# dronefreak/CABiNet

Measured on AMD Instinct MI355X. Metric: 1024x1024 images/sec fwd+bwd (CABiNet-MobileNetV3-Large), higher is better.
Workload: dtype f32; 1 GPU; BASELINE configs[2]: CABiNet-MobileNetV3-Large, 8x3x1024x1024 synthetic 8-class per GPU, fwd + 2x OhemCE + bwd + grad all-reduce + SGD step, HIP CAB/FFM kernels, fp32, random-init (model seed 0, gamma=0.5); per_gpu_batch=8, global_batch=8, n_classes=8, parallelism=dp1, miopen_find_mode=FAST

## Files before the change

cabinet_amd/csrc/conv3x3_s2.hip:

```cpp
#include "common.hpp"
#include "slab_sum.hpp"

namespace cabinet {

struct C3Shape {
    int B, H, W, Ho, Wo;
};

static C3Shape c3_shape(int B, int H, int W) { return C3Shape{B, H, W, (H - 1) / 2 + 1, (W - 1) / 2 + 1}; }

constexpr int CW_C = 64;
constexpr int CW_TW = 32;
constexpr int CW_IW = 2 * CW_TW + 1;
constexpr int CW_XP = 3 * CW_IW;
constexpr int CW_DLD = CW_TW + 1;
constexpr int CW_SLAB = CW_C * CW_C * 9;
constexpr int CW_TARGET_WG = 512;
constexpr int CW_MIN_ROWS = 4;

struct C3Plan {
    int tiles_x, strips, rows_per;
};

static C3Plan cw_plan(const C3Shape& s) {
    C3Plan p;
    p.tiles_x = ceil_div(s.Wo, CW_TW);
    const long per = (long)s.B * p.tiles_x;
    long strips = CW_TARGET_WG / per;
    const int cap = ceil_div(s.Ho, CW_MIN_ROWS);
    if (strips > cap) strips = cap;
    if (strips < 1) strips = 1;
    p.rows_per = ceil_div(s.Ho, (int)strips);
    p.strips = ceil_div(s.Ho, p.rows_per);
    return p;
}

__global__ __launch_bounds__(256, 2) void conv3x3s2_wgrad64_kernel(const float* __restrict__ dy, const float* __restrict__ x,
                                                                 C3Shape s, int tiles_x, int strips, int rows_per,
                                                                 float* __restrict__ slabs) {
    extern __shared__ __attribute__((aligned(16))) float smem[];
    float* xs = smem;
    float* dys = xs + CW_C * CW_XP;
    const int tid = threadIdx.x, wave = tid >> 6, lane = tid & 63, li = lane & 31, h = lane >> 5;
    int bi = blockIdx.x;
    const int tx = bi % tiles_x;
    bi /= tiles_x;
    const int strip = bi % strips, b = bi / strips;
    const int oy_begin = strip * rows_per, oy_end = min(s.Ho, oy_begin + rows_per);
    const int ox0 = tx * CW_TW, ix0 = 2 * ox0 - 1;
    const int ch = wave & 1, cj = wave >> 1;

    f32x16 acc[9];
#pragma unroll
    for (int t = 0; t < 9; ++t)
#pragma unroll
        for (int r = 0; r < 16; ++r) acc[t][r] = 0.f;

    const float* xb = x + (size_t)b * CW_C * s.H * s.W;
    const float* dyb = dy + (size_t)b * CW_C * s.Ho * s.Wo;
    const float* arow = dys + (32 * ch + li) * CW_DLD + h;
    const float* brow = xs + (32 * cj + li) * CW_XP + 2 * h;
    for (int oy = oy_begin; oy < oy_end; ++oy) {
        const int iy0 = 2 * oy - 1;
        __syncthreads();
        for (int i = tid; i < CW_C * CW_XP; i += 256) {
            const int ci = i / CW_XP, r = i - ci * CW_XP, yy = r / CW_IW, xx = r - yy * CW_IW;
            const int iy = iy0 + yy, ix = ix0 + xx;
            xs[i] = (iy >= 0 && iy < s.H && ix >= 0 && ix < s.W) ? xb[((size_t)ci * s.H + iy) * s.W + ix] : 0.f;
        }
        for (int i = tid; i < CW_C * CW_TW; i += 256) {
            const int co = i >> 5, c = i & 31, ox = ox0 + c;
            dys[co * CW_DLD + c] = ox < s.Wo ? dyb[((size_t)co * s.Ho + oy) * s.Wo + ox] : 0.f;
        }
        __syncthreads();
#pragma unroll
        for (int c0 = 0; c0 < CW_TW; c0 += 2) {
            const float a = arow[c0];
#pragma unroll
            for (int ky = 0; ky < 3; ++ky)
#pragma unroll
                for (int kx = 0; kx < 3; ++kx)
                    acc[3 * ky + kx] = mfma32(a, brow[ky * CW_IW + 2 * c0 + kx], acc[3 * ky + kx]);
        }
    }
    float* slab = slabs + (size_t)blockIdx.x * CW_SLAB;
#pragma unroll
    for (int r = 0; r < 16; ++r) {
        const int co = 32 * ch + acc_row(r) + 4 * h, ci = 32 * cj + li;
        float* p = slab + (co * CW_C + ci) * 9;
#pragma unroll
        for (int t = 0; t < 9; ++t) p[t] = acc[t][r];
    }
}

constexpr int CF_CI = 3, CF_CO = 16, CF_KK = CF_CI * 9;
constexpr int CF_TH = 4, CF_TW = 32;
constexpr int CF_IH = 2 * CF_TH + 1, CF_IW = 2 * CF_TW + 1;
constexpr int CF_PATCH = CF_CI * CF_IH * CF_IW;
constexpr int CF_DLD = CF_TH * CF_TW + 1;
constexpr int CF_SLAB = CF_CO * CF_KK;

__global__ __launch_bounds__(256) void conv3x3s2_wgrad_3_16_kernel(const float* __restrict__ dy, const float* __restrict__ x,
                                                                  C3Shape s, int tiles_x, float* __restrict__ slabs) {
    __shared__ __attribute__((aligned(16))) float dys[32 * CF_DLD];
    __shared__ float xs[CF_PATCH];
    __shared__ float red[4][CF_CO][32];
    const int tid = threadIdx.x, wave = tid >> 6, lane = tid & 63, li = lane & 31, h = lane >> 5;
    const int strips_y = (s.Ho + CF_TH - 1) / CF_TH;
    const int b = blockIdx.x / strips_y, oy0 = (blockIdx.x - b * strips_y) * CF_TH;
    const int kk = li < CF_KK ? li : 0;
    const int ko = ((kk / 9) * CF_IH + (kk % 9) / 3) * CF_IW + kk % 3;
    f32x16 acc;
#pragma unroll
    for (int r = 0; r < 16; ++r) acc[r] = 0.f;
    for (int i = tid; i < 16 * CF_DLD; i += 256) dys[16 * CF_DLD + i] = 0.f;
    const float* xb = x + (size_t)b * CF_CI * s.H * s.W;
    const float* dyb = dy + (size_t)b * CF_CO * s.Ho * s.Wo;
    const int iy0 = 2 * oy0 - 1;
    for (int t = 0; t < tiles_x; ++t) {
        const int ox0 = t * CF_TW, ix0 = 2 * ox0 - 1;
        __syncthreads();
        for (int i = tid; i < CF_PATCH; i += 256) {
            const int ci = i / (CF_IH * CF_IW), r = i - ci * CF_IH * CF_IW, yy = r / CF_IW, xx = r - yy * CF_IW;
            const int iy = iy0 + yy, ix = ix0 + xx;
            xs[i] = (iy >= 0 && iy < s.H && ix >= 0 && ix < s.W) ? xb[((size_t)ci * s.H + iy) * s.W + ix] : 0.f;
        }
        for (int i = tid; i < CF_CO * CF_TH * CF_TW; i += 256) {
            const int co = i / (CF_TH * CF_TW), p = i - co * (CF_TH * CF_TW), r = p / CF_TW, c = p - r * CF_TW;
            const int oy = oy0 + r, ox = ox0 + c;
            dys[co * CF_DLD + p] = (oy < s.Ho && ox < s.Wo) ? dyb[((size_t)co * s.Ho + oy) * s.Wo + ox] : 0.f;
        }
        __syncthreads();
        const float* drow = dys + li * CF_DLD + 32 * wave + h;
        const float* prow = xs + ko + 2 * wave * CF_IW + 2 * h;
#pragma unroll
        for (int c0 = 0; c0 < 32; c0 += 2) acc = mfma32(drow[c0], prow[2 * c0], acc);
    }
#pragma unroll
    for (int r = 0; r < 16; ++r) {
        const int co = acc_row(r) + 4 * h;
        if (co < CF_CO) red[wave][co][li] = acc[r];
    }
    __syncthreads();
    float* slab = slabs + (size_t)blockIdx.x * CF_SLAB;
    for (int i = tid; i < CF_SLAB; i += 256) {
        const int co = i / CF_KK, k = i - co * CF_KK;
        slab[i] = ((red[0][co][k] + red[1][co][k]) + red[2][co][k]) + red[3][co][k];
    }
}

typedef float f32x4v __attribute__((ext_vector_type(4)));
__device__ __forceinline__ f32x4v mfma16(float a, float b, f32x4v c) { return __builtin_amdgcn_mfma_f32_16x16x4f32(a, b, c, 0, 0, 0); }

constexpr int CD_NT = 64;
constexpr int CD_RP = 72;
constexpr int CD_CP = 2 * CD_RP;

__host__ __device__ constexpr int cd_par(int k) { return k == 1 ? 0 : 1; }
__host__ __device__ constexpr int cd_shift(int k) { return k == 0 ? 1 : 0; }

__global__ __launch_bounds__(256, 2) void conv3x3s2_dgrad64_kernel(const float* __restrict__ dy, const float* __restrict__ w,
                                                                 C3Shape s, int tiles_n, int strips, int rows_per,
                                                                 float* __restrict__ dx) {
    __shared__ __attribute__((aligned(16))) float dys[CW_C * CD_CP];
    const int tid = threadIdx.x, wave = tid >> 6, lane = tid & 63, lc = lane & 15, lk = lane >> 4;
    int bi = blockIdx.x;
    const int tn = bi % tiles_n;
    bi /= tiles_n;
    const int strip = bi % strips, b = bi / strips;
    const int m_begin = strip * rows_per, m_end = min(s.Ho, m_begin + rows_per);
    const int n0 = tn * CD_NT;
    const int ci0 = 16 * wave;

    float wr[9][16];
#pragma unroll
    for (int t = 0; t < 9; ++t)
#pragma unroll
        for (int ks = 0; ks < 16; ++ks) wr[t][ks] = w[((4 * ks + lk) * CW_C + ci0 + lc) * 9 + t];

    const float* dyb = dy + (size_t)b * CW_C * s.Ho * s.Wo;
    float* dxb = dx + ((size_t)b * CW_C + ci0 + 4 * lk) * s.H * s.W;
    const float* brow = dys + lk * CD_CP + lc;
    const bool pair_ok = (s.W & 1) == 0;
    for (int m = m_begin; m < m_end; ++m) {
        __syncthreads();
        for (int i = tid; i < CW_C * 2 * (CD_NT + 1); i += 256) {
            const int co = i / (2 * (CD_NT + 1)), r = i - co * 2 * (CD_NT + 1), rr = r / (CD_NT + 1), c = r - rr * (CD_NT + 1);
            const int oy = m + rr, ox = n0 + c;
            dys[co * CD_CP + rr * CD_RP + c] = (oy < s.Ho && ox < s.Wo) ? dyb[((size_t)co * s.Ho + oy) * s.Wo + ox] : 0.f;
        }
        __syncthreads();
#pragma unroll 1
        for (int ng = 0; ng < CD_NT / 16 && n0 + 16 * ng < s.Wo; ++ng) {
            f32x4v acc[2][2];
#pragma unroll
            for (int i = 0; i < 2; ++i)
#pragma unroll
                for (int j = 0; j < 2; ++j) acc[i][j] = f32x4v{0.f, 0.f, 0.f, 0.f};
            const float* bp = brow + 16 * ng;
#pragma unroll
            for (int ky = 0; ky < 3; ++ky)
#pragma unroll
                for (int kx = 0; kx < 3; ++kx) {
                    f32x4v p0 = {0.f, 0.f, 0.f, 0.f}, p1 = {0.f, 0.f, 0.f, 0.f};
                    const float* bt = bp + cd_shift(ky) * CD_RP + cd_shift(kx);
#pragma unroll
                    for (int ks = 0; ks < 16; ks += 2) {
                        p0 = mfma16(wr[3 * ky + kx][ks], bt[4 * ks * CD_CP], p0);
                        p1 = mfma16(wr[3 * ky + kx][ks + 1], bt[4 * (ks + 1) * CD_CP], p1);
                    }
                    acc[cd_par(ky)][cd_par(kx)] += p0 + p1;
                }
            const int ix = 2 * (n0 + 16 * ng + lc);
#pragma unroll
            for (int rp = 0; rp < 2; ++rp) {
                const int iy = 2 * m + rp;
                if (iy < s.H && ix < s.W) {
#pragma unroll
                    for (int r = 0; r < 4; ++r) {
                        float* p = dxb + ((size_t)r * s.H + iy) * s.W + ix;
                        if (pair_ok) {
                            *reinterpret_cast<f32x2*>(p) = f32x2{acc[rp][0][r], acc[rp][1][r]};
                        } else {
                            p[0] = acc[rp][0][r];
                            if (ix + 1 < s.W) p[1] = acc[rp][1][r];
                        }
                    }
                }
            }
        }
    }
}

bool conv3x3s2_supported(int Ci, int Co) { return (Ci == CW_C && Co == CW_C) || (Ci == CF_CI && Co == CF_CO); }

static C3Plan cd_plan(const C3Shape& s) {
    C3Plan p;
    p.tiles_x = ceil_div(s.Wo, CD_NT);
    const long per = (long)s.B * p.tiles_x;
    long strips = CW_TARGET_WG / per;
    if (strips > s.Ho) strips = s.Ho;
    if (strips < 1) strips = 1;
    p.rows_per = ceil_div(s.Ho, (int)strips);
    p.strips = ceil_div(s.Ho, p.rows_per);
    return p;
}

long long conv3x3s2_dgrad_workgroups(int B, int H, int W) {
    const C3Shape s = c3_shape(B, H, W);
    const long long per = (long long)B * ceil_div(s.Wo, CD_NT);
    if (per > (1ll << 30)) return per;
    const C3Plan p = cd_plan(s);
    return per * p.strips;
}

hipError_t conv3x3s2_dgrad_run(const float* dy, const float* w, int B, int H, int W, float* dx, hipStream_t stream) {
    const C3Shape s = c3_shape(B, H, W);
    const C3Plan p = cd_plan(s);
    hipLaunchKernelGGL(conv3x3s2_dgrad64_kernel, dim3(B * p.tiles_x * p.strips), dim3(256), 0, stream, dy, w, s, p.tiles_x,
                       p.strips, p.rows_per, dx);
    return hipGetLastError();
}

long long conv3x3s2_wgrad_slabs(int B, int Ci, int H, int W) {
    const C3Shape s = c3_shape(B, H, W);
    if (Ci == CF_CI) return (long long)B * ceil_div(s.Ho, CF_TH);
    const long long tiles_x = ceil_div(s.Wo, CW_TW);
    if ((long long)B * tiles_x > (1ll << 30)) return (long long)B * tiles_x;
    const C3Plan p = cw_plan(s);
    return (long long)B * p.tiles_x * p.strips;
}

size_t conv3x3s2_wgrad_workspace(int B, int Ci, int H, int W) {
    return align_up((size_t)conv3x3s2_wgrad_slabs(B, Ci, H, W) * (Ci == CF_CI ? CF_SLAB : CW_SLAB) * sizeof(float), 256);
}

hipError_t conv3x3s2_wgrad_run(const float* dy, const float* x, int B, int Ci, int H, int W, float* dw, void* ws,
                               hipStream_t stream) {
    const C3Shape s = c3_shape(B, H, W);
    float* slabs = static_cast<float*>(ws);
    const int nslab = (int)conv3x3s2_wgrad_slabs(B, Ci, H, W);
    if (Ci == CF_CI) {
        hipLaunchKernelGGL(conv3x3s2_wgrad_3_16_kernel, dim3(nslab), dim3(256), 0, stream, dy, x, s, ceil_div(s.Wo, CF_TW),
                           slabs);
    } else {
        const C3Plan p = cw_plan(s);
        const size_t lds = (size_t)(CW_C * CW_XP + CW_C * CW_DLD) * sizeof(float);
        static lds_attr_mask mask{0};
        if (hipError_t e = ensure_dynamic_lds(reinterpret_cast<const void*>(conv3x3s2_wgrad64_kernel), lds, mask); e != hipSuccess)
            return e;
        hipLaunchKernelGGL(conv3x3s2_wgrad64_kernel, dim3(nslab), dim3(256), lds, stream, dy, x, s, p.tiles_x, p.strips,
                           p.rows_per, slabs);
    }
    hipError_t e = hipGetLastError();
    if (e != hipSuccess) return e;
    slab_sum_launch(slabs, nslab, Ci == CF_CI ? CF_SLAB : CW_SLAB, dw, stream);
    return hipGetLastError();
}

}
```

cabinet_amd/csrc/stem_conv.hip:

```cpp
#include "act.hpp"
#include "common.hpp"
#include "slab_sum.hpp"

namespace cabinet {

constexpr int ST_K = 7, ST_S = 2, ST_PAD = 3, ST_CI = 3, ST_CO = 64;
constexpr int ST_KK = ST_CI * ST_K * ST_K;
constexpr int ST_KP = 148;
constexpr int ST_WLD = 149;

__host__ __device__ constexpr int stem_koff(int k, int IH, int IW) {
    return k < ST_KK ? ((k / (ST_K * ST_K)) * IH + (k % (ST_K * ST_K)) / ST_K) * IW + (k % ST_K) : 0;
}

struct StemShape {
    int B, H, W, Ho, Wo;
};

constexpr int SF_TH = 8, SF_TW = 32;
constexpr int SF_IH = (SF_TH - 1) * ST_S + ST_K;
constexpr int SF_IW = (SF_TW - 1) * ST_S + ST_K;
constexpr int SF_PATCH = ST_CI * SF_IH * SF_IW;

__global__ __launch_bounds__(256) void stem_conv_fwd_kernel(const float* __restrict__ x, const float* __restrict__ wgt,
                                                             StemShape s, int tiles_x, float* __restrict__ y) {
    extern __shared__ __attribute__((aligned(16))) float smem[];
    float* wl = smem;
    float* xs = wl + ST_CO * ST_WLD;
    const int tid = threadIdx.x, wave = tid >> 6, lane = tid & 63, li = lane & 31, h = lane >> 5;
    const int strips_y = (s.Ho + SF_TH - 1) / SF_TH;
    const int b = blockIdx.x / strips_y, oy0 = (blockIdx.x - b * strips_y) * SF_TH;
    for (int i = tid; i < ST_CO * ST_KP; i += 256) {
        const int co = i / ST_KP, k = i - co * ST_KP;
        wl[co * ST_WLD + k] = k < ST_KK ? wgt[co * ST_KK + k] : 0.f;
    }
    const float* xb = x + (size_t)b * ST_CI * s.H * s.W;
    const int iy0 = oy0 * ST_S - ST_PAD;
    const int poff0 = (ST_S * (2 * wave)) * SF_IW + ST_S * li, poff1 = poff0 + ST_S * SF_IW;
    for (int t = 0; t < tiles_x; ++t) {
        const int ox0 = t * SF_TW, ix0 = ox0 * ST_S - ST_PAD;
        __syncthreads();
        for (int i = tid; i < SF_PATCH; i += 256) {
            const int ci = i / (SF_IH * SF_IW), r = i - ci * SF_IH * SF_IW, yy = r / SF_IW, xx = r - yy * SF_IW;
            const int iy = iy0 + yy, ix = ix0 + xx;
            xs[i] = (iy >= 0 && iy < s.H && ix >= 0 && ix < s.W) ? xb[((size_t)ci * s.H + iy) * s.W + ix] : 0.f;
        }
        __syncthreads();
        f32x16 acc[2][2];
#pragma unroll
        for (int i = 0; i < 2; ++i)
#pragma unroll
            for (int j = 0; j < 2; ++j)
#pragma unroll
                for (int r = 0; r < 16; ++r) acc[i][j][r] = 0.f;
        const float* wrow = wl + li * ST_WLD + h;
        const float* xp0 = xs + poff0;
        const float* xp1 = xs + poff1;
#pragma unroll
        for (int k0 = 0; k0 < ST_KP; k0 += 2) {
            const int ko = h ? stem_koff(k0 + 1, SF_IH, SF_IW) : stem_koff(k0, SF_IH, SF_IW);
            const float a0 = wrow[k0], a1 = wrow[32 * ST_WLD + k0];
            const float b0 = xp0[ko], b1 = xp1[ko];
            acc[0][0] = mfma32(a0, b0, acc[0][0]);
            acc[0][1] = mfma32(a0, b1, acc[0][1]);
            acc[1][0] = mfma32(a1, b0, acc[1][0]);
            acc[1][1] = mfma32(a1, b1, acc[1][1]);
        }
        const int ox = ox0 + li;
#pragma unroll
        for (int j = 0; j < 2; ++j) {
            const int oy = oy0 + 2 * wave + j;
            if (oy < s.Ho && ox < s.Wo) {
#pragma unroll
                for (int i = 0; i < 2; ++i)
#pragma unroll
                    for (int r = 0; r < 16; ++r) {
                        const int co = 32 * i + acc_row(r) + 4 * h;
                        y[(((size_t)b * ST_CO + co) * s.Ho + oy) * s.Wo + ox] = acc[i][j][r];
                    }
            }
        }
    }
}

constexpr int SW_TH = 4, SW_TW = 32;
constexpr int SW_IH = (SW_TH - 1) * ST_S + ST_K;
constexpr int SW_IW = (SW_TW - 1) * ST_S + ST_K;
constexpr int SW_PATCH = ST_CI * SW_IH * SW_IW;
constexpr int SW_DLD = SW_TH * SW_TW + 1;
constexpr int SW_KB = 5;
constexpr int SW_G = ST_CO * SW_TH * (SW_TW / 4) / 256;
constexpr int SW_ROWS = ST_CI * SW_IH;
constexpr int SW_PR = (SW_ROWS + 3) / 4;
constexpr int SW_EXTRA = SW_ROWS * (SW_IW - 64);
constexpr int SW_BNP = 8;

struct StemBn {
    const float *z, *mean, *invstd, *weight, *bias, *coef;
};

template <typename T>
__device__ __forceinline__ T sw_ld(const float* base, unsigned byte_off) {
    return *reinterpret_cast<const T*>(reinterpret_cast<const char*>(base) + byte_off);
}

template <bool BN, bool VEC, int PJ>
__global__ __launch_bounds__(256, 2) void stem_conv_wrw_kernel(const float* __restrict__ dy, const float* __restrict__ x, StemBn bn,
                                                                StemShape s, int tiles_x, float* __restrict__ slabs) {
    extern __shared__ __attribute__((aligned(16))) float smem[];
    float* dys = smem;
    float* xs = dys + ST_CO * SW_DLD;
    float* bnp = xs + SW_PATCH;
    const int tid = threadIdx.x, wave = __builtin_amdgcn_readfirstlane(tid >> 6), lane = tid & 63, li = lane & 31, h = lane >> 5;
    const int strips_y = (s.Ho + SW_TH - 1) / SW_TH;
    const int b = blockIdx.x / strips_y, oy0 = (blockIdx.x - b * strips_y) * SW_TH;
    int ko[SW_KB];
#pragma unroll
    for (int kb = 0; kb < SW_KB; ++kb) {
        const int k = 32 * kb + li, kk = k < ST_KK ? k : 0;
        const int ci = kk / (ST_K * ST_K), r = kk - ci * ST_K * ST_K, ky = r / ST_K, kx = r - ky * ST_K;
        ko[kb] = (ci * SW_IH + ky) * SW_IW + kx;
    }
    f32x16 acc[2][SW_KB];
#pragma unroll
    for (int i = 0; i < 2; ++i)
#pragma unroll
        for (int j = 0; j < SW_KB; ++j)
#pragma unroll
            for (int r = 0; r < 16; ++r) acc[i][j][r] = 0.f;
    const float* xb = x + (size_t)b * ST_CI * s.H * s.W;
    const float* dyb = dy + (size_t)b * ST_CO * s.Ho * s.Wo;
    const float* zb = BN ? bn.z + (size_t)b * ST_CO * s.Ho * s.Wo : nullptr;
    const int iy0 = oy0 * ST_S - ST_PAD;
    if (BN && tid < ST_CO) {
        const float mu = bn.mean[tid], inv = bn.invstd[tid], gam = bn.weight[tid];
        float* q = bnp + tid * SW_BNP;
        q[0] = mu, q[1] = inv, q[2] = gam, q[3] = bn.bias[tid], q[4] = bn.coef[tid], q[5] = bn.coef[ST_CO + tid], q[6] = gam * inv;
    }
    const int gco = tid >> 5, gr = (tid >> 3) & 3, gc = (tid & 7) * 4;
    const bool grow_ok = oy0 + gr < s.Ho;
    const size_t gcs = (size_t)8 * s.Ho * s.Wo;
    const unsigned grow = ((unsigned)gco * s.Ho + min(oy0 + gr, s.Ho - 1)) * s.Wo;
    float* gdst = dys + gco * SW_DLD + gr * SW_TW + gc;
    int prow[SW_PR];
#pragma unroll
    for (int jj = 0; jj < SW_PR; ++jj) {
        const int rr = min(SW_PR * wave + jj, SW_ROWS - 1), ci = rr / SW_IH, iy = iy0 + rr - ci * SW_IH;
        prow[jj] = __builtin_amdgcn_readfirstlane((iy >= 0 && iy < s.H) ? (ci * s.H + iy) * s.W : -1);
    }
    struct Extra {
        int lds, col, row;
    };
    auto extra = [&]() {
        int te = tid;
        asm volatile("" : "+v"(te));
        const int i = min(te, SW_EXTRA - 1), er = i / (SW_IW - 64), ec = 64 + i - er * (SW_IW - 64);
        const int eci = er / SW_IH, eiy = iy0 + er - eci * SW_IH;
        return Extra{er * SW_IW + ec, ec, (eiy >= 0 && eiy < s.H) ? (eci * s.H + eiy) * s.W : -1};
    };

    f32x4 pg[SW_G], pz[SW_G];
    float pp[SW_PR + 1];
    auto request_dy = [&](int t, int j0, int j1) {
        const int ox = t * SW_TW + gc;
        if (VEC) {
            const unsigned o = (grow + min(ox, s.Wo - 4)) * 4u;
#pragma unroll
            for (int j = j0; j < j1; ++j) {
                pg[j] = sw_ld<f32x4>(dyb + j * gcs, o);
                if (BN) pz[j] = sw_ld<f32x4>(zb + j * gcs, o);
            }
        } else {
#pragma unroll
            for (int e = 0; e < 4; ++e) {
                const unsigned o = (grow + min(ox + e, s.Wo - 1)) * 4u;
#pragma unroll
                for (int j = j0; j < j1; ++j) {
                    pg[j][e] = sw_ld<float>(dyb + j * gcs, o);
                    if (BN) pz[j][e] = sw_ld<float>(zb + j * gcs, o);
                }
            }
        }
    };
    auto commit_dy = [&](int t, int j0, int j1) {
        const int ox = t * SW_TW + gc;
#pragma unroll
        for (int j = j0; j < j1; ++j) {
            f32x4 v = pg[j];
            if (BN) {
                const float* q = bnp + (gco + 8 * j) * SW_BNP;
                const float mu = q[0], inv = q[1], gam = q[2], bet = q[3], m1 = q[4], m2 = q[5], gi = q[6];
#pragma unroll
                for (int e = 0; e < 4; ++e) {
                    const float xh = (pz[j][e] - mu) * inv;
                    const float du = v[e] * act_grad(fmaf(xh, gam, bet), ACT_RELU);
                    v[e] = gi * (du - m1 - xh * m2);
                }
            }
#pragma unroll
            for (int e = 0; e < 4; ++e)
                gdst[j * 8 * SW_DLD + e] = (grow_ok && ox + e < s.Wo) ? v[e] : 0.f;
            if (BN) __builtin_amdgcn_sched_barrier(0);
        }
    };
    auto request_patch = [&](int t) {
        const int ix0 = t * SW_TW * ST_S - ST_PAD;
        const unsigned ixc = min(max(ix0 + lane, 0), s.W - 1) * 4u;
#pragma unroll
        for (int jj = 0; jj < SW_PR; ++jj) pp[jj] = sw_ld<float>(xb + max(prow[jj], 0), ixc);
        const Extra x5 = extra();
        pp[SW_PR] = sw_ld<float>(xb, (max(x5.row, 0) + min(max(ix0 + x5.col, 0), s.W - 1)) * 4u);
    };
    auto commit_patch = [&](int t) {
        const int ix0 = t * SW_TW * ST_S - ST_PAD;
        const bool okx = ix0 + lane >= 0 && ix0 + lane < s.W;
#pragma unroll
        for (int jj = 0; jj < SW_PR; ++jj)
            xs[min(SW_PR * wave + jj, SW_ROWS - 1) * SW_IW + lane] = (prow[jj] >= 0 && okx) ? pp[jj] : 0.f;
        const Extra x5 = extra();
        if (tid < SW_EXTRA) xs[x5.lds] = (x5.row >= 0 && ix0 + x5.col >= 0 && ix0 + x5.col < s.W) ? pp[SW_PR] : 0.f;
    };

    request_dy(0, 0, PJ);
    request_patch(0);
    for (int t = 0; t < tiles_x; ++t) {
        __syncthreads();
        commit_patch(t);
        commit_dy(t, 0, PJ);
        if (PJ < SW_G) {
            __builtin_amdgcn_sched_barrier(0);
            request_dy(t, PJ, PJ + 2);
            commit_dy(t, PJ, PJ + 2);
            __builtin_amdgcn_sched_barrier(0);
            request_dy(t, PJ + 2, SW_G);
            commit_dy(t, PJ + 2, SW_G);
        }
        __syncthreads();
        if (t + 1 < tiles_x) {
            request_dy(t + 1, 0, PJ);
            request_patch(t + 1);
        }
        const float* drow = dys + li * SW_DLD + 32 * wave + h;
        const int prow0 = (ST_S * wave) * SW_IW;
#pragma unroll 2
        for (int c0 = 0; c0 < 32; c0 += 2) {
            const float a0 = drow[c0], a1 = drow[32 * SW_DLD + c0];
            const int poff = prow0 + ST_S * (c0 + h);
#pragma unroll
            for (int kb = 0; kb < SW_KB; ++kb) {
                const float bv = xs[ko[kb] + poff];
                acc[0][kb] = mfma32(a0, bv, acc[0][kb]);
                acc[1][kb] = mfma32(a1, bv, acc[1][kb]);
            }
        }
    }
    __syncthreads();
    float* red = smem;
    constexpr int RLD = 161;
    int tid_e = tid;
    asm volatile("" : "+v"(tid_e));
    const int li_e = tid_e & 31, h_e = (tid_e >> 5) & 1;
    for (int w = 0; w < 4; ++w) {
        if (wave == w) {
#pragma unroll
            for (int i = 0; i < 2; ++i)
#pragma unroll
                for (int kb = 0; kb < SW_KB; ++kb)
#pragma unroll
                    for (int r = 0; r < 16; ++r) {
                        const int co = 32 * i + acc_row(r) + 4 * h_e, k = 32 * kb + li_e;
                        float* p = red + co * RLD + k;
                        *p = (w == 0) ? acc[i][kb][r] : *p + acc[i][kb][r];
                    }
        }
        __syncthreads();
    }
    float* slab = slabs + (size_t)blockIdx.x * ST_CO * ST_KK;
    for (int i = tid_e; i < ST_CO * ST_KK; i += 256) {
        const int co = i / ST_KK, k = i - co * ST_KK;
        slab[i] = red[co * RLD + k];
    }
}

static StemShape stem_shape(int B, int H, int W) {
    return StemShape{B, H, W, (H + 2 * ST_PAD - ST_K) / ST_S + 1, (W + 2 * ST_PAD - ST_K) / ST_S + 1};
}

size_t stem_conv_wrw_workspace(int B, int H, int W) {
    const StemShape s = stem_shape(B, H, W);
    return align_up((size_t)B * ceil_div(s.Ho, SW_TH) * ST_CO * ST_KK * sizeof(float), 256);
}

hipError_t stem_conv_fwd_run(const float* x, const float* w, int B, int H, int W, float* y, hipStream_t stream) {
    const StemShape s = stem_shape(B, H, W);
    const size_t lds = ((size_t)ST_CO * ST_WLD + SF_PATCH) * sizeof(float);
    static bool attr = false;
    if (!attr) {
        hipError_t e = hipFuncSetAttribute(reinterpret_cast<const void*>(stem_conv_fwd_kernel),
                                           hipFuncAttributeMaxDynamicSharedMemorySize, (int)lds);
        if (e != hipSuccess) return e;
        attr = true;
    }
    hipLaunchKernelGGL(stem_conv_fwd_kernel, dim3(B * ceil_div(s.Ho, SF_TH)), dim3(256), lds, stream, x, w, s,
                       ceil_div(s.Wo, SF_TW), y);
    return hipGetLastError();
}

constexpr int SW_PJ_PLAIN = 8, SW_PJ_BN = 4, SW_PJ_BN_RAGGED = 2;

template <bool BN>
static hipError_t stem_wrw_launch(const float* dy, const float* x, const StemBn& bn, int B, int H, int W, float* dw, float* slabs,
                                  hipStream_t stream) {
    const StemShape s = stem_shape(B, H, W);
    const int nslab = B * ceil_div(s.Ho, SW_TH), tiles_x = ceil_div(s.Wo, SW_TW);
    const size_t lds = ((size_t)ST_CO * SW_DLD + SW_PATCH + (BN ? ST_CO * SW_BNP : 0)) * sizeof(float);
    constexpr int PJ = BN ? SW_PJ_BN : SW_PJ_PLAIN, PJR = BN ? SW_PJ_BN_RAGGED : SW_PJ_PLAIN;
    const bool vec = (s.Wo & 3) == 0 && ((reinterpret_cast<uintptr_t>(dy) | reinterpret_cast<uintptr_t>(bn.z)) & 15) == 0;
    if (vec)
        hipLaunchKernelGGL((stem_conv_wrw_kernel<BN, true, PJ>), dim3(nslab), dim3(256), lds, stream, dy, x, bn, s, tiles_x, slabs);
    else
        hipLaunchKernelGGL((stem_conv_wrw_kernel<BN, false, PJR>), dim3(nslab), dim3(256), lds, stream, dy, x, bn, s, tiles_x, slabs);
    hipError_t e = hipGetLastError();
    if (e != hipSuccess) return e;
    slab_sum_launch(slabs, nslab, ST_CO * ST_KK, dw, stream);
    return hipGetLastError();
}

hipError_t stem_conv_wrw_run(const float* dy, const float* x, int B, int H, int W, float* dw, void* ws,
                             hipStream_t stream) {
    return stem_wrw_launch<false>(dy, x, StemBn{}, B, H, W, dw, static_cast<float*>(ws), stream);
}

size_t stem_conv_bn_bwd_workspace(int B, int H, int W) {
    const StemShape s = stem_shape(B, H, W);
    return bn_act_workspace(B, ST_CO, s.Ho * s.Wo) + stem_conv_wrw_workspace(B, H, W);
}

hipError_t stem_conv_bn_bwd_run(const float* g, const float* z, const float* x, const float* bn_weight, const float* bn_bias,
                                const float* save_mean, const float* save_invstd, int B, int H, int W, int training, float* dw,
                                float* dbn_weight, float* dbn_bias, void* ws, hipStream_t stream) {
    const StemShape s = stem_shape(B, H, W);
    const float* coef = nullptr;
    hipError_t e = bn_act_bwd_stats_run(g, z, bn_weight, bn_bias, save_mean, save_invstd, B, ST_CO, s.Ho * s.Wo, ACT_RELU, training,
                                        dbn_weight, dbn_bias, ws, &coef, stream);
    if (e != hipSuccess) return e;
    float* slabs = reinterpret_cast<float*>(static_cast<char*>(ws) + bn_act_workspace(B, ST_CO, s.Ho * s.Wo));
    return stem_wrw_launch<true>(g, x, StemBn{z, save_mean, save_invstd, bn_weight, bn_bias, coef}, B, H, W, dw, slabs, stream);
}

}
```

Baseline: 382.0 images/s.

## Software-pipeline global loads into LDS for stem fwd and 3x3 s2 dgrad convs

Both the stem 7x7 forward conv and the 3x3 stride-2 dgrad kernel now prefetch the next input tile or row into registers while MFMAs run on the current one, then commit it to LDS. This hides global-load latency behind compute. The dgrad kernel uses a 3-slot rotating LDS row buffer, so each output row loads only one new dy row instead of two. Both kernels also double-buffer their LDS operand reads around sched_barriers. The trade-off is higher register pressure, plus launch_bounds(256,2) on the stem kernel, which could spill.

```diff
diff --git a/cabinet_amd/csrc/conv3x3_s2.hip b/cabinet_amd/csrc/conv3x3_s2.hip
--- a/cabinet_amd/csrc/conv3x3_s2.hip
+++ b/cabinet_amd/csrc/conv3x3_s2.hip
@@ -153,8 +153,14 @@
 __device__ __forceinline__ f32x4v mfma16(float a, float b, f32x4v c) { return __builtin_amdgcn_mfma_f32_16x16x4f32(a, b, c, 0, 0, 0); }
 
 constexpr int CD_NT = 64;
-constexpr int CD_RP = 72;
-constexpr int CD_CP = 2 * CD_RP;
+constexpr int CD_RP = 80;
+constexpr int CD_SLOTS = 3;
+constexpr int CD_CP = CD_SLOTS * CD_RP;
+constexpr int CD_PR = CW_C / 4;
+
+__device__ __forceinline__ float cd_ld(const float* base, unsigned byte_off) {
+    return *reinterpret_cast<const float*>(reinterpret_cast<const char*>(base) + byte_off);
+}
 
 __host__ __device__ constexpr int cd_par(int k) { return k == 1 ? 0 : 1; }
 __host__ __device__ constexpr int cd_shift(int k) { return k == 0 ? 1 : 0; }
@@ -163,7 +169,7 @@
                                                                  C3Shape s, int tiles_n, int strips, int rows_per,
                                                                  float* __restrict__ dx) {
     __shared__ __attribute__((aligned(16))) float dys[CW_C * CD_CP];
-    const int tid = threadIdx.x, wave = tid >> 6, lane = tid & 63, lc = lane & 15, lk = lane >> 4;
+    const int tid = threadIdx.x, wave = __builtin_amdgcn_readfirstlane(tid >> 6), lane = tid & 63, lc = lane & 15, lk = lane >> 4;
     int bi = blockIdx.x;
     const int tn = bi % tiles_n;
     bi /= tiles_n;
@@ -182,14 +188,36 @@
     float* dxb = dx + ((size_t)b * CW_C + ci0 + 4 * lk) * s.H * s.W;
     const float* brow = dys + lk * CD_CP + lc;
     const bool pair_ok = (s.W & 1) == 0;
+    const unsigned colo = (unsigned)min(n0 + lane, s.Wo - 1) * 4u;
+    const bool col_ok = n0 + lane < s.Wo, halo_ok = n0 + CD_NT < s.Wo;
+    float pp[CD_PR + 1];
+    auto request = [&](int r) {
+        const int oy = min(r, s.Ho - 1);
+#pragma unroll
+        for (int j = 0; j < CD_PR; ++j) pp[j] = cd_ld(dyb + ((size_t)(CD_PR * wave + j) * s.Ho + oy) * s.Wo, colo);
+        int te = tid;
+        asm volatile("" : "+v"(te));
+        pp[CD_PR] = dyb[((size_t)min(te, CW_C - 1) * s.Ho + oy) * s.Wo + min(n0 + CD_NT, s.Wo - 1)];
+    };
+    auto commit = [&](int r, int slot) {
+        const bool row_ok = r < s.Ho;
+        float* d = dys + slot * CD_RP;
+#pragma unroll
+        for (int j = 0; j < CD_PR; ++j) d[(CD_PR * wave + j) * CD_CP + lane] = (row_ok && col_ok) ? pp[j] : 0.f;
+        if (tid < CW_C) d[tid * CD_CP + CD_NT] = (row_ok && halo_ok) ? pp[CD_PR] : 0.f;
+    };
+    request(m_begin);
+    commit(m_begin, 0);
+    request(m_begin + 1);
+    int s0 = 0;
     for (int m = m_begin; m < m_end; ++m) {
-        __syncthreads();
-        for (int i = tid; i < CW_C * 2 * (CD_NT + 1); i += 256) {
-            const int co = i / (2 * (CD_NT + 1)), r = i - co * 2 * (CD_NT + 1), rr = r / (CD_NT + 1), c = r - rr * (CD_NT + 1);
-            const int oy = m + rr, ox = n0 + c;
-            dys[co * CD_CP + rr * CD_RP + c] = (oy < s.Ho && ox < s.Wo) ? dyb[((size_t)co * s.Ho + oy) * s.Wo + ox] : 0.f;
-        }
-        __syncthreads();
+        const int s1 = s0 == CD_SLOTS - 1 ? 0 : s0 + 1;
+        commit(m + 1, s1);
+        __syncthreads();
+        if (m + 1 < m_end) request(m + 2);
+        const float* bp0 = brow + s0 * CD_RP;
+        const float* bp1 = brow + s1 * CD_RP;
+        s0 = s1;
 #pragma unroll 1
         for (int ng = 0; ng < CD_NT / 16 && n0 + 16 * ng < s.Wo; ++ng) {
             f32x4v acc[2][2];
@@ -197,20 +225,28 @@
             for (int i = 0; i < 2; ++i)
 #pragma unroll
                 for (int j = 0; j < 2; ++j) acc[i][j] = f32x4v{0.f, 0.f, 0.f, 0.f};
-            const float* bp = brow + 16 * ng;
-#pragma unroll
-            for (int ky = 0; ky < 3; ++ky)
-#pragma unroll
-                for (int kx = 0; kx < 3; ++kx) {
-                    f32x4v p0 = {0.f, 0.f, 0.f, 0.f}, p1 = {0.f, 0.f, 0.f, 0.f};
-                    const float* bt = bp + cd_shift(ky) * CD_RP + cd_shift(kx);
-#pragma unroll
-                    for (int ks = 0; ks < 16; ks += 2) {
-                        p0 = mfma16(wr[3 * ky + kx][ks], bt[4 * ks * CD_CP], p0);
-                        p1 = mfma16(wr[3 * ky + kx][ks + 1], bt[4 * (ks + 1) * CD_CP], p1);
-                    }
-                    acc[cd_par(ky)][cd_par(kx)] += p0 + p1;
+            float bv[2][8];
+            auto read_half = [&](int g, float* v) {
+                const int t = g / 2;
+                const float* bt = (cd_shift(t / 3) ? bp1 : bp0) + 16 * ng + cd_shift(t % 3);
+#pragma unroll
+                for (int i = 0; i < 8; ++i) v[i] = bt[4 * (8 * (g % 2) + i) * CD_CP];
+            };
+            read_half(0, bv[0]);
+            f32x4v p0, p1;
+#pragma unroll
+            for (int g = 0; g < 18; ++g) {
+                const int t = g / 2, k8 = 8 * (g % 2);
+                if (g + 1 < 18) read_half(g + 1, bv[(g + 1) & 1]);
+                if (g % 2 == 0) p0 = p1 = f32x4v{0.f, 0.f, 0.f, 0.f};
+#pragma unroll
+                for (int i = 0; i < 8; i += 2) {
+                    p0 = mfma16(wr[t][k8 + i], bv[g & 1][i], p0);
+                    p1 = mfma16(wr[t][k8 + i + 1], bv[g & 1][i + 1], p1);
                 }
+                if (g % 2 == 1) acc[cd_par(t / 3)][cd_par(t % 3)] += p0 + p1;
+                __builtin_amdgcn_sched_barrier(0);
+            }
             const int ix = 2 * (n0 + 16 * ng + lc);
 #pragma unroll
             for (int rp = 0; rp < 2; ++rp) {
diff --git a/cabinet_amd/csrc/stem_conv.hip b/cabinet_amd/csrc/stem_conv.hip
--- a/cabinet_amd/csrc/stem_conv.hip
+++ b/cabinet_amd/csrc/stem_conv.hip
@@ -17,35 +17,81 @@
     int B, H, W, Ho, Wo;
 };
 
+template <typename T>
+__device__ __forceinline__ T sw_ld(const float* base, unsigned byte_off) {
+    return *reinterpret_cast<const T*>(reinterpret_cast<const char*>(base) + byte_off);
+}
+
 constexpr int SF_TH = 8, SF_TW = 32;
 constexpr int SF_IH = (SF_TH - 1) * ST_S + ST_K;
 constexpr int SF_IW = (SF_TW - 1) * ST_S + ST_K;
 constexpr int SF_PATCH = ST_CI * SF_IH * SF_IW;
-
-__global__ __launch_bounds__(256) void stem_conv_fwd_kernel(const float* __restrict__ x, const float* __restrict__ wgt,
-                                                             StemShape s, int tiles_x, float* __restrict__ y) {
+constexpr int SF_ROWS = ST_CI * SF_IH;
+constexpr int SF_PR = (SF_ROWS + 3) / 4;
+constexpr int SF_XW = SF_IW - 64;
+constexpr int SF_EXTRA = SF_ROWS * SF_XW;
+constexpr int SF_XT = (SF_EXTRA + 255) / 256;
+constexpr int SF_KG = 2, SF_NG = ST_KP / (2 * SF_KG);
+static_assert(SF_NG * 2 * SF_KG == ST_KP, "k-groups tile the contraction");
+
+__global__ __launch_bounds__(256, 2) void stem_conv_fwd_kernel(const float* __restrict__ x, const float* __restrict__ wgt,
+                                                                StemShape s, int tiles_x, float* __restrict__ y) {
     extern __shared__ __attribute__((aligned(16))) float smem[];
     float* wl = smem;
     float* xs = wl + ST_CO * ST_WLD;
-    const int tid = threadIdx.x, wave = tid >> 6, lane = tid & 63, li = lane & 31, h = lane >> 5;
+    const int tid = threadIdx.x, wave = __builtin_amdgcn_readfirstlane(tid >> 6), lane = tid & 63, li = lane & 31, h = lane >> 5;
     const int strips_y = (s.Ho + SF_TH - 1) / SF_TH;
     const int b = blockIdx.x / strips_y, oy0 = (blockIdx.x - b * strips_y) * SF_TH;
+    const float* xb = x + (size_t)b * ST_CI * s.H * s.W;
+    const int iy0 = oy0 * ST_S - ST_PAD;
+    int prow[SF_PR];
+#pragma unroll
+    for (int jj = 0; jj < SF_PR; ++jj) {
+        const int rr = min(SF_PR * wave + jj, SF_ROWS - 1), ci = rr / SF_IH, iy = iy0 + rr - ci * SF_IH;
+        prow[jj] = __builtin_amdgcn_readfirstlane((iy >= 0 && iy < s.H) ? ci * s.H + iy : -1);
+    }
+    int xlds[SF_XT], xcol[SF_XT], xrow[SF_XT];
+#pragma unroll
+    for (int e = 0; e < SF_XT; ++e) {
+        const int i = min(tid + 256 * e, SF_EXTRA - 1), er = i / SF_XW, ci = er / SF_IH, iy = iy0 + er - ci * SF_IH;
+        xcol[e] = 64 + i - er * SF_XW;
+        xlds[e] = er * SF_IW + xcol[e];
+        xrow[e] = (iy >= 0 && iy < s.H) ? ci * s.H + iy : -1;
+    }
+    float pp[SF_PR + SF_XT];
+    auto request = [&](int t) {
+        const int ix0 = t * SF_TW * ST_S - ST_PAD;
+        const unsigned ixc = min(max(ix0 + lane, 0), s.W - 1) * 4u;
+#pragma unroll
+        for (int jj = 0; jj < SF_PR; ++jj) pp[jj] = sw_ld<float>(xb + (size_t)max(prow[jj], 0) * s.W, ixc);
+#pragma unroll
+        for (int e = 0; e < SF_XT; ++e)
+            pp[SF_PR + e] = xb[(size_t)max(xrow[e], 0) * s.W + min(max(ix0 + xcol[e], 0), s.W - 1)];
+    };
+    auto commit = [&](int t) {
+        const int ix0 = t * SF_TW * ST_S - ST_PAD;
+        const bool okx = ix0 + lane >= 0 && ix0 + lane < s.W;
+#pragma unroll
+        for (int jj = 0; jj < SF_PR; ++jj)
+            xs[min(SF_PR * wave + jj, SF_ROWS - 1) * SF_IW + lane] = (prow[jj] >= 0 && okx) ? pp[jj] : 0.f;
+#pragma unroll
+        for (int e = 0; e < SF_XT; ++e)
+            if (tid + 256 * e < SF_EXTRA)
+                xs[xlds[e]] = (xrow[e] >= 0 && ix0 + xcol[e] >= 0 && ix0 + xcol[e] < s.W) ? pp[SF_PR + e] : 0.f;
+    };
+
+    request(0);
     for (int i = tid; i < ST_CO * ST_KP; i += 256) {
         const int co = i / ST_KP, k = i - co * ST_KP;
         wl[co * ST_WLD + k] = k < ST_KK ? wgt[co * ST_KK + k] : 0.f;
     }
-    const float* xb = x + (size_t)b * ST_CI * s.H * s.W;
-    const int iy0 = oy0 * ST_S - ST_PAD;
-    const int poff0 = (ST_S * (2 * wave)) * SF_IW + ST_S * li, poff1 = poff0 + ST_S * SF_IW;
+    commit(0);
+    __syncthreads();
+    const int poff0 = (ST_S * (2 * wave)) * SF_IW + ST_S * li;
+    const size_t ylane = (((size_t)b * ST_CO + 4 * h) * s.Ho + oy0 + 2 * wave) * s.Wo + li;
     for (int t = 0; t < tiles_x; ++t) {
-        const int ox0 = t * SF_TW, ix0 = ox0 * ST_S - ST_PAD;
-        __syncthreads();
-        for (int i = tid; i < SF_PATCH; i += 256) {
-            const int ci = i / (SF_IH * SF_IW), r = i - ci * SF_IH * SF_IW, yy = r / SF_IW, xx = r - yy * SF_IW;
-            const int iy = iy0 + yy, ix = ix0 + xx;
-            xs[i] = (iy >= 0 && iy < s.H && ix >= 0 && ix < s.W) ? xb[((size_t)ci * s.H + iy) * s.W + ix] : 0.f;
-        }
-        __syncthreads();
+        const int ox0 = t * SF_TW;
+        if (t + 1 < tiles_x) request(t + 1);
         f32x16 acc[2][2];
 #pragma unroll
         for (int i = 0; i < 2; ++i)
@@ -55,18 +101,38 @@
                 for (int r = 0; r < 16; ++r) acc[i][j][r] = 0.f;
         const float* wrow = wl + li * ST_WLD + h;
         const float* xp0 = xs + poff0;
-        const float* xp1 = xs + poff1;
-#pragma unroll
-        for (int k0 = 0; k0 < ST_KP; k0 += 2) {
-            const int ko = h ? stem_koff(k0 + 1, SF_IH, SF_IW) : stem_koff(k0, SF_IH, SF_IW);
-            const float a0 = wrow[k0], a1 = wrow[32 * ST_WLD + k0];
-            const float b0 = xp0[ko], b1 = xp1[ko];
-            acc[0][0] = mfma32(a0, b0, acc[0][0]);
-            acc[0][1] = mfma32(a0, b1, acc[0][1]);
-            acc[1][0] = mfma32(a1, b0, acc[1][0]);
-            acc[1][1] = mfma32(a1, b1, acc[1][1]);
+        float av[2][SF_KG][2], bv[2][SF_KG][2];
+        auto read_group = [&](int g, float(*a)[2], float(*bq)[2]) {
+#pragma unroll
+            for (int i = 0; i < SF_KG; ++i) {
+                const int k0 = 2 * (SF_KG * g + i);
+                const int kl = stem_koff(k0, SF_IH, SF_IW), d = stem_koff(k0 + 1, SF_IH, SF_IW) - kl;
+                const float* q = xp0 + (h ? d : 0);
+                a[i][0] = wrow[k0], a[i][1] = wrow[32 * ST_WLD + k0];
+                bq[i][0] = q[kl], bq[i][1] = q[kl + ST_S * SF_IW];
+            }
+        };
+        read_group(0, av[0], bv[0]);
+#pragma unroll
+        for (int g = 0; g < SF_NG; ++g) {
+            if (g + 1 < SF_NG) read_group(g + 1, av[(g + 1) & 1], bv[(g + 1) & 1]);
+#pragma unroll
+            for (int i = 0; i < SF_KG; ++i) {
+                const float a0 = av[g & 1][i][0], a1 = av[g & 1][i][1], b0 = bv[g & 1][i][0], b1 = bv[g & 1][i][1];
+                acc[0][0] = mfma32(a0, b0, acc[0][0]);
+                acc[0][1] = mfma32(a0, b1, acc[0][1]);
+                acc[1][0] = mfma32(a1, b0, acc[1][0]);
+                acc[1][1] = mfma32(a1, b1, acc[1][1]);
+            }
+            __builtin_amdgcn_sched_barrier(0);
+        }
+        if (t + 1 < tiles_x) {
+            __syncthreads();
+            commit(t + 1);
         }
         const int ox = ox0 + li;
+        size_t yo = ylane + ox0;
+        asm volatile("" : "+v"(yo));
 #pragma unroll
         for (int j = 0; j < 2; ++j) {
             const int oy = oy0 + 2 * wave + j;
@@ -74,12 +140,11 @@
 #pragma unroll
                 for (int i = 0; i < 2; ++i)
 #pragma unroll
-                    for (int r = 0; r < 16; ++r) {
-                        const int co = 32 * i + acc_row(r) + 4 * h;
-                        y[(((size_t)b * ST_CO + co) * s.Ho + oy) * s.Wo + ox] = acc[i][j][r];
-                    }
-            }
-        }
+                    for (int r = 0; r < 16; ++r)
+                        y[yo + ((size_t)(32 * i + acc_row(r)) * s.Ho + j) * s.Wo] = acc[i][j][r];
+            }
+        }
+        __syncthreads();
     }
 }
 
@@ -98,11 +163,6 @@
 struct StemBn {
     const float *z, *mean, *invstd, *weight, *bias, *coef;
 };
-
-template <typename T>
-__device__ __forceinline__ T sw_ld(const float* base, unsigned byte_off) {
-    return *reinterpret_cast<const T*>(reinterpret_cast<const char*>(base) + byte_off);
-}
 
 template <bool BN, bool VEC, int PJ>
 __global__ __launch_bounds__(256, 2) void stem_conv_wrw_kernel(const float* __restrict__ dy, const float* __restrict__ x, StemBn bn,
```

After: 388.6 images/s (median of 6 runs). 1.7% higher.
